# rrwick/Polypolish

Hardware: AMD Instinct MI355X
Metric: assembly Mbp polished/sec at 200x coverage; bit-identical FASTA vs reference (higher is better)
Workload: dtype u8/u32 counts + f64 depth

## Files before the change

### polypolish_amd/csrc/pp_internal.h

```cpp
#pragma once

#include <hip/hip_runtime.h>

#include <cstdarg>
#include <cstdint>
#include <cstdio>
#include <string>
#include <thread>
#include <vector>

#include "polypolish_hip.h"

#ifndef PP_MIRROR_REGISTRY_DECLARED
#define PP_MIRROR_REGISTRY_DECLARED
void pp_mirror_register_(const void *owner, const void *p, size_t bytes);
void pp_mirror_forget_(const void *owner);
bool pp_mirror_trusted_(const void *p, size_t bytes);
#endif

namespace pp {

constexpr int TILE = 2048;
constexpr int TILE_THREADS = 1024;
constexpr int COARSE_WINDOWS = 8;
// ... 122 lines not shown
    uint64_t acc_n = 0, acc_seq = 0, acc_cig = 0;
    uint64_t total_out = 0, n_multi = 0, n_keys = 0;
    uint64_t last_dev_error = ~0ull;
    std::vector<uint64_t> contig_out_off;
    std::vector<pp_contig_stats> stats;

    pp::DevBuf b_bases, b_contig_off, b_status;
    pp::DevBuf b_in[11];
    bool acc_wo = false;
    pp::DevBuf b_gstart, b_nkeep, b_aflag, b_hist, b_wincnt, b_winoff, b_entA, b_entB, b_ccnt, b_coff;
    pp::DevBuf b_code, b_winlen, b_winout, b_flag_pos, b_flag_cov, b_flag_scr, b_scratch;
    pp::DevBuf b_vote_tab;
    pp::DevBuf b_multi, b_meta, b_out, b_flag_bits, b_win_nflag, b_win_slab, b_slab_win, b_slabs, b_ents, b_keys, b_own;
    pp::DevBuf b_win_heavy, b_hslab;
    std::vector<uint64_t> wo_runs;
    pp::DevBuf b_runs, b_first, b_xcnt, b_xent, b_need_win, b_win_lo, b_win_hi;
    std::vector<uint32_t> runs_on_dev;
    size_t xcap = 0;
    bool no_direct = false;
    bool wo_untrusted = false;
    bool trust_all = false;
    bool no_wo = false;
    size_t xcap_limit = ~(size_t)0;
    uint32_t maxlen_hint = 0;
    bool last_direct = false;
    bool nothing_flagged_last = false;
    std::vector<uint32_t> emit;
    std::vector<uint32_t> run_full_of;
    uint32_t run_nc = 0;
    uint32_t last_multi = ~0u;
    uint32_t last_listed = ~0u;
// ... 73 lines not shown
```

### polypolish_amd/csrc/pp_k_direct.h

```cpp
#pragma once

#include "pp_wo_home.h"

namespace pp {

constexpr u32 NOHOME = 0xFFFFFFFFu;
__device__ __forceinline__ bool wo_bulk(bool contig_ok, u32 ref_start, u32 seq_len, u32 op0, u64 clen) {
    return contig_ok && op0 == ((seq_len << 4) | (u32)PP_OP_M) && seq_len > 0 && seq_len <= FAST_MAX_LEN && (u64)ref_start + seq_len <= clen;
}
__device__ __forceinline__ uint4 wo_item(u64 so, u32 len, u32 kc, u64 g, u32 w, u32 file_idx) {
    uint4 e;
    e.x = (u32)so;
    e.y = ((u32)(so >> 32) & 0xFFu) | (kc << 8) | (len << 24);
    e.z = (u32)(int)((long long)g - (long long)w * TILE) & 0x3FFFFFFFu;
    e.w = file_idx;
    return e;
}

constexpr u32 XLOCAL = 64, CTG_LDS = 1024;
struct CtgTab {
    const u64 *lds, *mem;
    bool in_lds;
    __device__ __forceinline__ u64 operator()(u32 i) const {
        u32 x, y;
        if (in_lds) {
            const u64 v = lds[i];
            x = (u32)v; y = (u32)(v >> 32);
            asm volatile("" : "+v"(x), "+v"(y));
        } else {
            const u64 v = mem[i];
            x = (u32)v; y = (u32)(v >> 32);
// ... 69 lines not shown
struct PrepdArgs {
    u64 n;
    const pp_wo_rec *wo;
    const u64 *cig_off;
    const u32 *n_cig, *cigar;
    const u8 *seq;
    const u64 *contig_off;
    u32 n_contigs, nwin;
    const u32 *run_end;
    u32 n_runs;
    u32 *first, *x_cnt, *x_nb;
    uint4 *xent;
    u32 xcap;
    u32 *maxlen;
    u64 *x_need;
    u64 unused_[3];
    u64 seq_bytes;
    u64 *status;
};

template <typename CTG>
__device__ __forceinline__ void general_record(const pp_wo_rec &r, const PrepdArgs &P, CTG ctg, const XSink &X) {
    u32 g_out = 0, nk_out = 0;
    u8 fl_out = 0;
    const u32 fi = r.file_idx;
    if (fi >= P.n) return;
    if (r.contig >= P.n_contigs) { report(P.status, fi, DE_BAD_CONTIG); return; }
    const u64 c_lo = ctg(r.contig), c_hi = ctg(r.contig + 1u);
    X.not_bulk(wo_home(c_lo, r.ref_start, P.nwin));
    {
        const bool multi = r.op0 == PP_WO_MULTI_RUN;
// ... 76 lines not shown
        if (lo < hi) {
            const pp_wo_rec r0 = wo[lo];
            if (r0.contig < n_contigs) wb = wo_home(P.contig_off[r0.contig], r0.ref_start, nwin);
        }
        s_wbase = wb;
    }
    XSink X{st_item, st_key, l_cnt, l_base, l_nb, &n_st, XSTAGE, 0u, P.xcap, P.x_cnt, P.x_nb, P.xent, P.x_need, status};
    X.clear();
    __syncthreads();
    PP_STAMP(0, 1);
    X.wbase = s_wbase;
    const CtgTab ctg{s_ctg, P.contig_off, ctg_lds};
    const u32 lane = threadIdx.x & 63u;
    const u32 stride = nwin + 1u;
    u32 *const first = P.first;
    auto fill = [&](bool want, u32 run, u32 from, u32 to, u32 val) {
        if (want && to - from < 4u) {
            for (u32 w = from; w <= to; w++) first[(u64)run * stride + w] = val;
            want = false;
        }
        u64 m = __ballot(want);
        while (m) {
            const int lead = __ffsll((long long)m) - 1;
            m &= m - 1;
            const u32 rr = (u32)__builtin_amdgcn_readlane((int)run, lead), ff = (u32)__builtin_amdgcn_readlane((int)from, lead),
                      tt = (u32)__builtin_amdgcn_readlane((int)to, lead), vv = (u32)__builtin_amdgcn_readlane((int)val, lead);
            for (u64 w = (u64)ff + lane; w <= tt; w += 64) first[(u64)rr * stride + w] = vv;
        }
    };
    u32 runw = 0, runw_lo = 0;
// ... 65 lines not shown
            const bool begins = valid && (starts || (hp != NOHOME && h > hp));
            const bool descent = valid && !starts && hp != NOHOME && h < hp;
            const bool ends = valid && (u32)a + 1u == run_hi;
            const bool bad = in && (file_idx >= n || k == 0 || seq_off + seq_len > (1ull << 40) || seq_off + seq_len > P.seq_bytes);
            if (__ballot(begins || descent || ends || bad)) {
                if (bad) {
                    if (file_idx >= n) report(status, a, DE_BAD_MIRROR);
                    else if (k == 0) report(status, file_idx, DE_BAD_K);
                    else if (seq_off + seq_len > (1ull << 40)) report(status, file_idx, DE_OVERFLOW);
                    else report(status, file_idx, DE_SEQ_RANGE);
                }
                if (descent) report(status, (1ull << 40) - 1ull, DE_MIRROR_ORDER);
                fill(begins, run, starts ? 0u : hp + 1u, h, (u32)a);
                fill(ends, run, h + 1u, nwin, (u32)a + 1u);
            }
            const u32 w1 = bulk ? (u32)((g + seq_len - 1u) / (u64)TILE) : 0u;
            if (bulk && w1 > h) X.emit(w1, wo_item(seq_off, seq_len, kclass_of(k), g, w1, file_idx));
            if (bulk) fast_len = max(fast_len, seq_len);
            else if (in) {
                const u32 slot = atomicAdd(&n_later, 1u);
                if (slot < LATER_MAX) { later[2u * slot] = qa[u]; later[2u * slot + 1u] = qb[u]; }
            }
            if (PP_PREPD_ROLL) ask(u, a0_next, more);
        }
        unit = unit_next;
    }
    PP_STAMP(0, 2);
    __syncthreads();
    PP_STAMP(0, 3);
    const u32 n_noted = n_later;
// ... 104 lines not shown
```

### polypolish_amd/csrc/pp_k_tile.h

```cpp
#pragma once

namespace pp {

struct TileArgs {
    const uint4 *entA;
    const u32 *win_off;
    u32 nwin;
    const u8 *seq;
    const u8 *seq4;
    const u64 *seq_off;
    const u64 *cig_off;
    const u32 *n_cig;
    const u32 *cigar;
    const u32 *kk;
    const u8 *bases;
    u64 G;
    const u64 *contig_off;
    u32 n_contigs;
    u32 min_depth;
    double fv, fi;
    u8 *code;
    u32 *win_len;
    u32 *win_coarse, *win_coarse2;
    u32 *counters;
// ... 23 lines not shown
    u64 *stamps;
#endif
    double *dbg_depth;
    u32 *dbg_counts;
    u8 *dbg_status;
    u64 *status;
    int dbg;
    const uint4 *wo;
    const u32 *first;
    u32 n_runs;
    u32 xcap;
    const u32 *x_cnt;
    const uint4 *xent;
    u32 *need_win;
    u64 *n_need;
};

struct RecMap {
    const u32 *pre;
    const u32 *first;
    u32 R;
    u32 v0, nv;
    u32 w;
    bool one_contig;
    u32 c0;
    u64 c_lo, clen;
    u32 w_in_contig;
};

struct TileShare {
    u32 b;
    u32 *any_shared;
    const u32 *kk;
    u32 *pt, *pt_over;
    const u32 *pmask;
};

__device__ __forceinline__ void share_range(u32 *cnt, u32 *ndbits, const TileShare &S, int p0, int p1, u32 kc, u32 rec) {
    if (kc == 0 || p1 <= p0) return;
    bool inexact;
    const u32 d = share_deficit(kc, S.b, S.kk, rec, &inexact);
    atomicAdd(&cnt[ROW_DEF * TILE + p0], d);
// ... 678 lines not shown
    const u32 nv_last = (u32)__builtin_amdgcn_readfirstlane((int)(nv ? nv - 1u : 0u));
    const u32 lo_w = 0u, hi_w = nv + nx;
    if (lo_w >= hi_w) return;
    auto rec_at = [&](u32 v) -> u32 {
        u32 a = M.first[0] + v;
        for (u32 r = 1; r < M.R; r++)
            if (v >= M.pre[r]) a = M.first[r] + (v - M.pre[r]);
        return a;
    };
    const uint4 *const wq = A.wo;
    auto index_of = [&](u32 u) -> u32 {
        if (REC && u < nv) return rec_at(M.v0 + r_lo + min(u, nv_last));
        const u32 x = x_lo + XS * (u - min(u, nv));
        return !REC && X.indirect ? X.indirect[x] : x;
    };
    auto words_at = [&](bool rec, u32 idx, uint4 &a, uint4 &b) {
        if (REC) {
            const uint4 *const p1 = rec ? wq + 2ull * idx : ent + idx, *const p2 = rec ? wq + 2ull * idx + 1 : ent + idx;
            a = *p1;
            b = *p2;
        } else a = ent[idx];
    };
    uint4 nxt, nxt2 = make_uint4(0, 0, 0, 0);
    {
        const u32 u = lo_w + min(lane, min(BATCH, hi_w - lo_w) - 1u);
        words_at(u < nv, index_of(u), nxt, nxt2);
    }
    for (u32 eb = lo_w; eb < hi_w; eb += BATCH) {
        const u32 nb = min(BATCH, hi_w - eb);
        uint4 my = nxt;
        bool rec_ok = true, is_rec = false;
        if (REC) {
            is_rec = eb + min(lane, nb - 1u) < nv;
            const uint4 qa = nxt, qb = nxt2;
            u64 c_lo = M.c_lo, clen = M.clen;
            bool c_ok = qa.x == M.c0;
            if (!M.one_contig) {
                const u32 cc = min(qa.x, A.n_contigs - 1u);
                c_lo = A.contig_off[cc];
                clen = A.contig_off[cc + 1] - c_lo;
                c_ok = qa.x < A.n_contigs;
            }
            rec_ok = !is_rec || wo_bulk(c_ok, qa.y, qa.w, qb.z, clen);
            const u32 kc = __ballot(is_rec && qa.z != 1u) ? kclass_of(qa.z) : 0u;
            uint4 made = wo_item((u64)qb.x | ((u64)qb.y << 32), qa.w, kc, c_lo + qa.y, M.w, qb.w);
            if (M.one_contig) made.z = (qa.y - M.w_in_contig) & 0x3FFFFFFFu;
            if (is_rec) my = made;
        }
        const bool more = eb + BATCH < hi_w;
        const u32 nxt_u = more ? eb + BATCH + min(lane, min(BATCH, hi_w - eb - BATCH) - 1u) : eb + min(lane, nb - 1u);
        const u32 nxt_idx = index_of(nxt_u);
        const bool nxt_rec = nxt_u < nv;
        auto ask_for_next = [&](u32 tie) {
            u32 idx = nxt_idx;
            asm volatile("" : "+v"(idx) : "v"(tie));
            words_at(nxt_rec, idx, nxt, nxt2);
        };
        if (!WIDE && more) ask_for_next(0u);
        const u32 my_flags = is_rec ? 0u : item_flags(my.y, my.z);
        bool my_slow = lane < nb && (my_flags & 3u) != 0;
        bool deferred = false;
        if (!REC && X.defer && __ballot(my_slow)) {
            if (my_slow) {
                const u32 slot = atomicAdd(X.defer_n, 1u);
                if (slot < X.defer_cap) {
                    X.defer[slot] = index_of(eb + lane);
                    deferred = true;
                    my_slow = false;
                }
            }
        }
// ... 113 lines not shown
    const u32 inc = wave_scan_incl(raw.len);
    const u32 total = (u32)__builtin_amdgcn_readlane((int)inc, (int)(R - 1u));
    B.pre_v = lane < R ? inc - raw.len : total;
    B.first_v = raw.f0;
    B.R = R;
    return B;
}
template <int NCH>
struct DirectBulk {
    static constexpr int GROUP_SPLIT = 5;
    BulkRuns B;
    u32 v0, nv, pm;
    const uint4 *items;
    u32 x0, nx, px;
    u32 pass;
    uint4 ea, eb;
    uint4 na, nb;
    uint4 W[NCH];
    u32 tail;
    static constexpr u32 WAVES = TILE_THREADS / 64;

    __device__ __forceinline__ u32 n_pass() const { return pm + px; }
    __device__ __forceinline__ u32 entry_of(u32 p, u32 lane) const {
        const u32 vs = v0 + 64u * p;
        const u32 v = min(vs + lane, v0 + nv - 1u);
        u32 r = 0;
        for (u32 j = 1; j < B.R; j++)
            if (vs >= (u32)__builtin_amdgcn_readlane((int)B.pre_v, (int)j)) r = j;
        u32 pr = (u32)__builtin_amdgcn_readlane((int)B.pre_v, (int)r), nx_ = (u32)__builtin_amdgcn_readlane((int)B.pre_v, (int)(r + 1u));
        u32 a = (u32)__builtin_amdgcn_readlane((int)B.first_v, (int)r) + (v - pr);
        while (__ballot(v >= nx_)) {
            r++;
            pr = nx_;
            nx_ = (u32)__builtin_amdgcn_readlane((int)B.pre_v, (int)(r + 1u));
            if (v >= pr) a = (u32)__builtin_amdgcn_readlane((int)B.first_v, (int)r) + (v - pr);
        }
        return a;
    }
    __device__ __forceinline__ void ask_sources(const TileArgs &A, u32 p, u32 lane, uint4 &qa, uint4 &qb) const {
        if (p < pm) {
            const u32 a = entry_of(p, lane);
            qa = A.wo[2ull * a];
            qb = A.wo[2ull * a + 1];
        } else {
            const u32 i = x0 + min(64u * (p - pm) + lane, nx - 1u);
            qa = items[i];
            qb = qa;
        }
    }
    __device__ __forceinline__ bool in_list(u32 p, u32 lane) const { return p < pm ? 64u * p + lane < nv : 64u * (p - pm) + lane < nx; }
    struct Lean {
        u64 so_l;
        u32 pack;
    };
    static constexpr u32 LN_REL0 = 256;
    static constexpr u32 LN_FAST = 1u << 20, LN_PLAIN = 1u << 21, LN_SHARED = 1u << 22, LN_NOTRIM = 1u << 23, LN_POINT = 1u << 24, LN_SLOW = 1u << 25;
    __device__ static __forceinline__ bool loadable(const TileArgs &A, u64 so, u32 L) {
        return L - 1u <= 32u * NCH - 1u && so + L >= 8u && so + 32u * NCH <= A.seq_bytes;
    }
    __device__ __forceinline__ Lean distill(const TileArgs &A, const RecMap &M, u32 p, const uint4 &qa, const uint4 &qb, bool listed) const {
        Lean n{0ull, 0u};
        if (p < pm) {
            const u32 ref_start = qa.y, L = qa.w;
            u32 c_lo32 = (u32)M.c_lo, clen32 = (u32)M.clen;
            bool c_ok = qa.x == M.c0;
            if (!M.one_contig) {
                const u32 cc = min(qa.x, A.n_contigs - 1u);
                const u64 lo64 = A.contig_off[cc];
                c_lo32 = (u32)lo64;
                clen32 = (u32)(A.contig_off[cc + 1] - lo64);
                c_ok = qa.x < A.n_contigs;
            }
            const u32 rel = c_lo32 + ref_start - (u32)((u64)M.w * TILE);
            const bool bulk = listed && c_ok && qb.z == ((L << 4) | (u32)PP_OP_M) && L - 1u < FAST_MAX_LEN && L <= clen32 && ref_start <= clen32 - L &&
                              rel < (u32)TILE;
            const u64 so = (u64)qb.x | ((u64)qb.y << 32);
            const bool plain = bulk && loadable(A, so, L);
            n.so_l = plain ? so : 0ull;
            n.pack = bulk ? ((rel + LN_REL0) | (L << 12) | LN_FAST | (plain ? LN_PLAIN : 0u) | (qa.z != 1u ? LN_SHARED : 0u)) : 0u;
        } else {
            const u32 ex = qa.x, ey = qa.y, ez = qa.z;
            const u32 flags = item_flags(ey, ez), L = ey >> 24;
            const bool slow = (flags & 3u) != 0, point = (flags & ENT_POINT) != 0, notrim = (flags & ENT_NOTRIM) != 0;
            const u64 so = (u64)ex | ((u64)(ey & 0xFFu) << 32);
            const int rel = item_rel(ez);
            const bool fast = listed && !slow && rel > -(int)LN_REL0 && rel < TILE;
            const bool plain = fast && !point && loadable(A, so, L) && wide4_takes(ex, ey, ez);
            n.so_l = plain ? so : 0ull;
            n.pack = listed ? (slow ? LN_SLOW : (fast ? (((u32)(rel + (int)LN_REL0)) | (L << 12) | LN_FAST | (plain ? LN_PLAIN : 0u) |
                                                         (((ey >> 8) & 0xFFu) ? LN_SHARED : 0u) | (notrim ? LN_NOTRIM : 0u) | (point ? LN_POINT : 0u))
                                                       : 0u))
                            : 0u;
        }
        return n;
    }
    __device__ __forceinline__ void begin(const TileArgs &A, const BulkRuns &runs, u32 v0_, u32 nv_, const uint4 *items_, u32 x0_, u32 nx_, u32 wave, u32 lane) {
        B = runs;
        v0 = v0_;
        nv = nv_;
        pm = (nv + 63u) >> 6;
        items = items_;
        x0 = x0_;
        nx = nx_;
        px = (nx + 63u) >> 6;
        pass = wave;
        ea = eb = make_uint4(0, 0, 0, 0);
        if (pass < n_pass()) ask_sources(A, pass, lane, ea, eb);
    }
    __device__ __forceinline__ void raw_place(const TileArgs &A, u32 p, const uint4 &qa, const uint4 &qb, u64 &so, u32 &L) const {
        if (p < pm) {
            so = (u64)qb.x | ((u64)qb.y << 32);
            L = qa.w;
        } else {
            so = (u64)qa.x | ((u64)(qa.y & 0xFFu) << 32);
            L = (qa.y & 0x00030000u) ? 0u : qa.y >> 24;
        }
    }
    __device__ __forceinline__ void stage(const TileArgs &A, u32 lane) {
        if (pass >= n_pass()) return;
        const bool more = pass + WAVES < n_pass();
        ask_sources(A, more ? pass + WAVES : pass, lane, na, nb);
        u64 so;
        u32 L;
        raw_place(A, pass, ea, eb, so, L);
        const bool ld = loadable(A, so, L);
        tail = load4_unaligned(A.seq4 + ((ld ? so + (L - 1u) : 7ull) >> 1) - 3);
        const u8 *const q = A.seq4 + ((ld ? so : 0ull) >> 1);
#pragma unroll
        for (int c = 0; c < NCH; c++) W[c] = load16_unaligned(q + 16 * c);
    }
    __device__ __forceinline__ void run(const TileArgs &A, u32 *cnt, u32 *ndbits, const TileShare &S, const u32 *asm_w, const u32 *asm4, const RecMap &M,
                                        u32 *defer, u32 *defer_n, u32 defer_cap, u32 lane) {
        const u32 np = n_pass();
        if (pass >= np) return;
        Lean cur = distill(A, M, pass, ea, eb, in_list(pass, lane));
        for (; pass < np; pass += WAVES) {
            const bool more = pass + WAVES < np;
            if (__ballot((cur.pack & (LN_SLOW | LN_POINT)) != 0 || (cur.pack & (LN_FAST | LN_PLAIN)) == LN_FAST)) {
                const int rel_r = (int)(cur.pack & 0xFFFu) - (int)LN_REL0;
                uint4 my;
                u32 src;
                if (pass < pm) {
                    src = entry_of(pass, lane);
                    const uint4 qa = A.wo[2ull * src], qb = A.wo[2ull * src + 1];
                    my = wo_item((u64)qb.x | ((u64)qb.y << 32), qa.w, kclass_of(qa.z), (u64)M.w * TILE + (u32)rel_r, M.w, qb.w);
                } else {
                    src = x0 + min(64u * (pass - pm) + lane, nx - 1u);
                    my = items[src];
                }
                if (cur.pack & LN_SLOW) {
// ... 1 lines not shown
                    if (slot < defer_cap) defer[slot] = src;
                }
                if ((cur.pack & LN_POINT) && rel_r >= 0) {
                    tile_add(cnt, (my.y >> 24) ? ROW_OTH : ROW_DEL, rel_r);
                    share_range(cnt, ndbits, S, rel_r, rel_r + 1, (my.y >> 8) & 0xFFu, my.w);
                    if ((my.y >> 24) == 2u) pt_insert(S.pt, S.pt_over, rel_r, A.seq, (u64)my.x | ((u64)(my.y & 0xFFu) << 32));
                }
                u64 rest = __ballot((cur.pack & (LN_FAST | LN_PLAIN | LN_POINT)) == LN_FAST);
                while (rest) {
                    const u32 j = (u32)__ffsll((long long)rest) - 1u;
                    rest &= rest - 1;
                    const FastItem f = fast_fetch(my, j, 64u, A.seq);
                    fast_apply(cnt, ndbits, S, asm_w, f, (u32)__builtin_amdgcn_readlane((int)my.w, (int)j), fast_load(A.seq, f, lane), lane);
                }
            }
            const Lean nxt = distill(A, M, pass + WAVES, na, nb, more && in_list(pass + WAVES, lane));
            if (pass + 2u * WAVES < np) ask_sources(A, pass + 2u * WAVES, lane, na, nb);
            const u32 tail_now = tail;
            const u8 *const q_next = A.seq4 + (nxt.so_l >> 1);
            const u8 *const t_next = A.seq4 + (((nxt.pack & LN_PLAIN) ? nxt.so_l + (((nxt.pack >> 12) & 0xFFu) - 1u) : 7ull) >> 1) - 3;

            const int rel = (int)(cur.pack & 0xFFFu) - (int)LN_REL0;
            const u32 L = (cur.pack >> 12) & 0xFFu;
            const bool plain = (cur.pack & LN_PLAIN) != 0;
            const u64 so = cur.so_l;
            const u32 adj = (u32)so & 1u;
            int nkeep = trim4(tail_now, so + (L - 1u), L);
            if (cur.pack & LN_NOTRIM) nkeep = (int)L;
            else if (plain && nkeep < 0) nkeep = trim_bytes(A.seq + so, L);
            const int lo = max(0, -rel), hi = min(nkeep, TILE - rel);
            const bool live = plain && hi > lo;
            if (live) {
// ... 221 lines not shown
        u32 inc = len;
        for (int o = 1; o < 32; o <<= 1) {
            const u32 t = (u32)__shfl_up((int)inc, o, 64);
            if ((int)r >= o) inc += t;
        }
        if (r <= R && r < 32u) s_run[r] = inc - len;
        if (r < R) s_run[32u + r] = f0;
        if (r == 63u) s_run[52] = min(A.x_cnt[w], A.xcap);
        if (r == 62u) s_run[53] = A.x_cnt[A.nwin + w];
    }
    if (tid >= 128u && tid < 128u + (u32)PMASK_WORDS) ((u32 *)s_dirty)[tid - 128u] = g_pmask_tab.v[tid - 128u];
    if (tid >= 64u && tid < 64u + PT_SLOTS * 3u) s_pt[tid - 64u] = 0;
    if (wave < 2u) {
        const u32 cw = find_contig_wave(A.contig_off, A.n_contigs, wave == 0 ? w0 : min(w0 + TILE, A.G) - 1, lane);
        if (lane == 0) { if (wave == 0) s_c0 = cw; else s_c1 = cw; }
        if (DIRECT && wave == 0 && lane == 0) {
            const u64 lo64 = A.contig_off[cw], len64 = A.contig_off[cw + 1] - lo64;
            s_run[48] = (u32)lo64; s_run[49] = (u32)(lo64 >> 32); s_run[50] = (u32)len64; s_run[51] = (u32)(len64 >> 32);
        }
    }
    if constexpr (BULK) D.stage(A, lane);
    __syncthreads();
    PP_STOP_AFTER(1)

#ifdef PP_TILE_STAMPS
    if (tid == 0) A.stamps[8ull * blockIdx.x + 6] = wall_clock64();
#endif
    u32 e0, e1, n_rec = 0, n_notbulk = 0;
    const uint4 *items;
    if (DIRECT) {
        e0 = 0;
        e1 = s_run[52];
        items = A.xent + (u64)w * A.xcap;
        n_rec = s_run[A.n_runs];
// ... 2 lines not shown
        e0 = A.win_off[w];
        e1 = A.win_off[w + 1];
        items = A.entA;
    }
    const TileShare S{win_fx_bits(e1 - e0 + n_rec - n_notbulk), &s_shared, A.kk, s_pt, &s_ptover, (const u32 *)s_dirty};
    {
        u32 i0 = e0, i1 = e1, v0 = 0, v1 = n_rec;
        if (heavy) {
            const u32 chunk = ((e1 - e0 + HEAVY_PARTS - 1u) / HEAVY_PARTS + 63u) & ~63u;
            i0 = min(e1, e0 + part * chunk);
            i1 = min(e1, i0 + chunk);
            const u32 vchunk = ((n_rec + HEAVY_PARTS - 1u) / HEAVY_PARTS + 63u) & ~63u;
            v0 = min(n_rec, part * vchunk);
            v1 = min(n_rec, v0 + vchunk);
        }
        const u32 c0 = (u32)__builtin_amdgcn_readfirstlane((int)s_c0);
        RecMap M{s_run, s_run + 32, A.n_runs, (u32)__builtin_amdgcn_readfirstlane((int)v0),
                 (u32)__builtin_amdgcn_readfirstlane((int)(v1 - v0)), w, s_c0 == s_c1, c0, 0, 0, 0};
        if (DIRECT) {
            M.c_lo = (u64)(u32)__builtin_amdgcn_readfirstlane((int)s_run[48]) | ((u64)(u32)__builtin_amdgcn_readfirstlane((int)s_run[49]) << 32);
            M.clen = (u64)(u32)__builtin_amdgcn_readfirstlane((int)s_run[50]) | ((u64)(u32)__builtin_amdgcn_readfirstlane((int)s_run[51]) << 32);
            M.w_in_contig = (u32)(w0 - M.c_lo);
        }
        constexpr u32 WAVES = TILE_THREADS / 64;
        if constexpr (BULK) {
            D.run(A, cnt, s_ndbits, S, asm_w, asm4, M, s_slow, &s_nslow, SLOW_CAP, lane);
            __syncthreads();
            const u32 n_slow = s_nslow;
            if (n_slow > SLOW_CAP) {
                const u32 n = i1 - i0;
                if (wave < n)
                    tile_items<GW, P4, false>(A, cnt, s_ndbits, S, asm_w, asm4, items, M, i0, i1,
                                              ItemList{i0 + wave, (n - wave - 1u) / WAVES + 1u, WAVES, nullptr, nullptr, nullptr, 0u, true}, wave, lane);
            } else if (wave < n_slow)
                tile_items<GW, P4, false>(A, cnt, s_ndbits, S, asm_w, asm4, items, M, i0, i1,
                                          ItemList{wave, (n_slow - wave - 1u) / WAVES + 1u, WAVES, s_slow, nullptr, nullptr, 0u, true}, wave, lane);
        } else {
            constexpr u32 IPP = (P4 && GW == 5) ? 1u : PlainCfg<GW>::IPP;
// ... 326 lines not shown
```

### polypolish_amd/csrc/pp_kernels.hip

```cpp
#include "pp_internal.h"

#include <algorithm>
#include <cstring>

#include "pp_k_common.h"
#include "pp_k_prep.h"
#include "pp_k_bucket.h"
#include "pp_k_direct.h"
#include "pp_k_tile.h"
#include "pp_k_exact.h"
#include "pp_k_emit.h"
#include "pp_k_debug.h"
#include <hip/hip_ext.h>

using namespace pp;

static bool env_is0(const char *name) { const char *v = getenv(name); return v && atoi(v) == 0; }
static bool env_on(const char *name) { const char *v = getenv(name); return v && atoi(v) != 0; }
static long env_num(const char *name, long dflt) { const char *v = getenv(name); return v ? atol(v) : dflt; }
struct Knobs {
    bool timer_record = env_on("PP_TIMER_RECORD");
    bool no_seq4 = env_is0("PP_SEQ4");
    bool no_wo = env_is0("PP_WO");
    bool no_direct = env_is0("PP_DIRECT");
// ... 548 lines not shown
    int rc;
#define ENS(buf, bytes) if ((rc = dev_ensure(ctx, ctx->buf, (size_t)(bytes)))) return rc
    ENS(b_meta, P.meta_words * 8);
    ENS(b_vote_tab, (size_t)VOTE_TAB_N * 8);
    ENS(b_win_heavy, nwin);
    ENS(b_hslab, (size_t)HEAVY_SLOTS * HEAVY_PARTS * HSLAB_WORDS * 4);
    if (!P.direct) { ENS(b_gstart, n * 4); ENS(b_nkeep, n * 4); }
    if (P.direct) {
        ENS(b_first, (uint64_t)P.n_runs * (nwin + 1) * 4);
        ENS(b_xcnt, nwin * 8);
        if (dev_ensure(ctx, ctx->b_xent, (size_t)(nwin * ctx->xcap * 16))) {
            (void)hipGetLastError();
            *no_room = true;
            return PP_OK;
        }
        ENS(b_need_win, nwin * 4); ENS(b_win_lo, nwin * 4); ENS(b_win_hi, nwin * 4);
        std::vector<uint32_t> ends(ctx->wo_runs.begin(), ctx->wo_runs.end());
        if (!(ends == ctx->runs_on_dev && ctx->b_runs.p)) {
            const void *dummy;
            ctx->runs_on_dev.clear();
            if ((rc = upload(ctx, ctx->b_runs, ends.data(), ends.size() * 4, &dummy))) return rc;
            PP_HIPCHK(ctx, hipStreamSynchronize(ctx->stream));
            ctx->runs_on_dev = ends;
        }
    }
    if (!P.direct) {
        ENS(b_hist, (uint64_t)P.NB * P.ncoarse * 4); ENS(b_wincnt, nwin * 4); ENS(b_winoff, (nwin + 1) * 4);
        ENS(b_ccnt, (uint64_t)P.ncoarse * 4); ENS(b_coff, ((uint64_t)P.ncoarse + 1) * 4);
        if (P.two_level) ENS(b_entB, ctx->cap_ent * 16);
    }
// ... 103 lines not shown
static void prep_direct(pp_ctx *ctx, const RunPlan &P, const RunDev &D) {
    const Knobs &K = knobs();
    const pp_aln_batch &B = ctx->dbatch;
    const uint64_t n = P.n;
    const u32 nwin = P.nwin;
    hipStream_t st = ctx->stream;
    const uint64_t noted_est = B.n_cig_total > n ? (B.n_cig_total - n) / 2 : 0;
    const uint64_t nbd_default = std::max<uint64_t>(std::max<uint64_t>(768, n / 8700), noted_est / 400);
    const uint32_t NBD = (uint32_t)std::max<uint64_t>(1, std::min<uint64_t>(K.prepd_blocks > 0 ? (uint64_t)K.prepd_blocks : nbd_default, (n + 2047) / 2048));
    const uint64_t chunk_d = (n + NBD - 1) / NBD;
    timer_begin(ctx, "prep");
    PrepdArgs PA{};
    PA.n = n; PA.wo = D.wo; PA.cig_off = (const u64 *)B.cig_off; PA.n_cig = B.n_cig; PA.cigar = B.cigar; PA.seq = B.seq;
    PA.contig_off = (const u64 *)ctx->b_contig_off.p; PA.n_contigs = P.nc_full; PA.nwin = nwin;
    PA.run_end = (const u32 *)ctx->b_runs.p; PA.n_runs = P.n_runs; PA.first = (u32 *)ctx->b_first.p;
    PA.x_cnt = (u32 *)ctx->b_xcnt.p; PA.x_nb = (u32 *)ctx->b_xcnt.p + nwin; PA.xent = (uint4 *)ctx->b_xent.p; PA.xcap = (u32)ctx->xcap;
    PA.maxlen = (u32 *)(D.meta + MW_MAXLEN); PA.x_need = D.meta + MW_X_NEED;
    PA.seq_bytes = B.seq_bytes;
    PA.status = D.status();
    if (K.prepd_threads == 1024) hipLaunchKernelGGL(k_prepd<1024>, dim3(NBD), dim3(1024), 0, st, (u64)chunk_d, PA);
    else hipLaunchKernelGGL(k_prepd<512>, dim3(NBD), dim3(512), 0, st, (u64)chunk_d, PA);
    timer_end(ctx);
    timer_begin(ctx, "bucket");
    hipLaunchKernelGGL(k_winplan, dim3((nwin + 255) / 256), dim3(256), 0, st, nwin, P.n_runs, (const u32 *)ctx->b_first.p,
                       (const u32 *)ctx->b_xcnt.p, (const u32 *)ctx->b_xcnt.p + nwin, (u32)ctx->xcap, P.heavy_min, D.heavy, (u8 *)ctx->b_win_heavy.p,
                       D.meta + MW_ITEMS, D.status());
    timer_end(ctx);
}

static void prep_bucketing(pp_ctx *ctx, const RunPlan &P, const RunDev &D) {
    const pp_aln_batch &B = ctx->dbatch;
// ... 87 lines not shown
    T.flag_pos = (u32 *)ctx->b_flag_pos.p; T.flag_cov = (u32 *)ctx->b_flag_cov.p;
    T.flag_bits = (u32 *)ctx->b_flag_bits.p; T.win_nflag = (u32 *)ctx->b_win_nflag.p;
    T.win_slab = (u32 *)ctx->b_win_slab.p; T.slab_win = (u32 *)ctx->b_slab_win.p; T.slabs = (u32 *)ctx->b_slabs.p; T.cap_slabs = (u32)ctx->cap_slabs;
    T.stats = (ContigStatsDev *)(D.meta + meta_stats_at(P.nc));
    T.maxlen = (const u32 *)(D.meta + MW_MAXLEN);
    T.scr_need = D.meta + MW_SCR_NEED;
    T.flag_scr = (u64 *)ctx->b_flag_scr.p;
    T.seq_bytes = B.seq_bytes;
    T.own = D.own;
    T.own_win = D.own_win;
    T.heavy = D.heavy; T.win_heavy = (u8 *)ctx->b_win_heavy.p; T.hslab = (u32 *)ctx->b_hslab.p;
    T.dbg_depth = (double *)ctx->b_dbg_depth.p; T.dbg_counts = (u32 *)ctx->b_dbg_counts.p;
    T.dbg_status = (u8 *)ctx->b_dbg_status.p; T.status = D.status();
    T.dbg = ctx->debug ? (ctx->debug_level == 3 ? 3 : (knobs().debug_replay2 ? 2 : 1)) : 0;
    T.wo = (const uint4 *)D.wo; T.first = (const u32 *)ctx->b_first.p; T.n_runs = P.n_runs; T.xcap = (u32)ctx->xcap;
    T.x_cnt = (const u32 *)ctx->b_xcnt.p; T.xent = (const uint4 *)ctx->b_xent.p; T.need_win = (u32 *)ctx->b_need_win.p; T.n_need = D.meta + MW_N_NEED;
    return T;
}

static int launch_tile(pp_ctx *ctx, const RunPlan &P, TileArgs &T) {
    hipStream_t st = ctx->stream;
    hipEvent_t ev_start = nullptr, ev_stop = nullptr;
    const bool ev_launch = timer_for_launch(ctx, "tile", &ev_start, &ev_stop);
    if (!ev_launch) timer_begin(ctx, "tile");
#ifdef PP_TILE_STAMPS
    static DevBuf b_stamps;
    const size_t stamp_bytes = (size_t)(HEAVY_BLOCKS + P.per * 8) * 64;
    if (int rc2 = dev_ensure(ctx, b_stamps, stamp_bytes)) return rc2;
    PP_HIPCHK(ctx, hipMemsetAsync(b_stamps.p, 0, stamp_bytes, st));
    T.stamps = (u64 *)b_stamps.p;
#endif
// ... 671 lines not shown

extern "C" void pp_ctx_destroy(pp_ctx *ctx) {
    if (!ctx) return;
    if (pp_ctx_wait(ctx) != PP_OK) {
        delete ctx;
        return;
    }
    pp_comm_destroy(ctx);
    (void)hipSetDevice(ctx->device);
    (void)hipStreamSynchronize(ctx->stream);
    DevBuf *all[] = {&ctx->b_comm, &ctx->b_gather, &ctx->b_bases, &ctx->b_contig_off, &ctx->b_status, &ctx->b_gstart, &ctx->b_nkeep,
                     &ctx->b_aflag, &ctx->b_hist, &ctx->b_wincnt, &ctx->b_winoff, &ctx->b_entA, &ctx->b_entB, &ctx->b_ccnt, &ctx->b_coff,
                     &ctx->b_code, &ctx->b_winlen, &ctx->b_winout, &ctx->b_flag_pos, &ctx->b_flag_cov,
                     &ctx->b_flag_scr, &ctx->b_scratch, &ctx->b_multi, &ctx->b_meta, &ctx->b_vote_tab, &ctx->b_flag_bits, &ctx->b_win_nflag, &ctx->b_win_slab, &ctx->b_slab_win, &ctx->b_slabs, &ctx->b_ents, &ctx->b_keys, &ctx->b_own,
                     &ctx->b_win_heavy, &ctx->b_hslab, &ctx->b_sub_bases,
                     &ctx->b_runs, &ctx->b_first, &ctx->b_xcnt, &ctx->b_xent, &ctx->b_need_win, &ctx->b_win_lo, &ctx->b_win_hi,
                     &ctx->b_out, &ctx->b_emit_done, &ctx->b_wincoarse, &ctx->b_dbg_depth, &ctx->b_dbg_counts, &ctx->b_dbg_status,
                     &ctx->b_dfmt_idx, &ctx->b_dfmt_rec, &ctx->b_dfmt_names, &ctx->b_dfmt_noff, &ctx->b_dfmt_emit, &ctx->b_dfmt_len,
                     &ctx->b_dfmt_bsum, &ctx->b_dfmt_boff, &ctx->b_dfmt_res, &ctx->b_dfmt_stage,
                     &ctx->f_refend[0], &ctx->f_refend[1], &ctx->f_pass[0], &ctx->f_pass[1], &ctx->f_orient, &ctx->f_poisoned,
                     &ctx->f_insert, &ctx->f_list, &ctx->f_blkcnt, &ctx->f_thr};
    for (DevBuf *b : all) dev_free(*b);
    for (auto &b : ctx->b_in) dev_free(b);
    for (auto &b : ctx->b_split) dev_free(b);
    for (auto &f : ctx->f_in) for (auto &b : f) dev_free(b);
    for (auto &b : ctx->f_rec) dev_free(b);
    timers_release(ctx);
    if (ctx->h_meta) (void)hipHostFree(ctx->h_meta);
    for (hipEvent_t e : ctx->event_pool) (void)hipEventDestroy(e);
    (void)hipStreamDestroy(ctx->stream);
    delete ctx;
// ... 46 lines not shown
```

Before: 18410.

## Precompute packed per-alignment source words in direct pass for tile kernel

The direct pass now writes a compact 8-byte source word per alignment that packs the sequence offset, window-relative position, length, and bulk/shared/far/tail flags. The tile kernel reads this word instead of two 16-byte alignment records plus contig offset lookups, which removes per-record contig bounds checks and the per-tile contig metadata in RecMap. This cuts global memory traffic and ALU work in the hot tile loop. In exchange it adds one extra buffer write per alignment in the direct pass, and shared (k!=1) records still do a gather for kclass and file index.

```diff
diff --git a/polypolish_amd/csrc/pp_internal.h b/polypolish_amd/csrc/pp_internal.h
--- a/polypolish_amd/csrc/pp_internal.h
+++ b/polypolish_amd/csrc/pp_internal.h
@@ -160,7 +160,7 @@
     pp::DevBuf b_multi, b_meta, b_out, b_flag_bits, b_win_nflag, b_win_slab, b_slab_win, b_slabs, b_ents, b_keys, b_own;
     pp::DevBuf b_win_heavy, b_hslab;
     std::vector<uint64_t> wo_runs;
-    pp::DevBuf b_runs, b_first, b_xcnt, b_xent, b_need_win, b_win_lo, b_win_hi;
+    pp::DevBuf b_runs, b_first, b_xcnt, b_xent, b_src, b_need_win, b_win_lo, b_win_hi;
     std::vector<uint32_t> runs_on_dev;
     size_t xcap = 0;
     bool no_direct = false;
diff --git a/polypolish_amd/csrc/pp_k_direct.h b/polypolish_amd/csrc/pp_k_direct.h
--- a/polypolish_amd/csrc/pp_k_direct.h
+++ b/polypolish_amd/csrc/pp_k_direct.h
@@ -15,6 +15,19 @@
     e.z = (u32)(int)((long long)g - (long long)w * TILE) & 0x3FFFFFFFu;
     e.w = file_idx;
     return e;
+}
+constexpr u32 SRC_REL_AT = 8, SRC_LEN_AT = 19, SRC_FAR_BYTES = 256;
+constexpr u32 SRC_BULK = 1u << 27;
+constexpr u32 SRC_SHARED = 1u << 28;
+constexpr u32 SRC_FAR = 1u << 29;
+constexpr u32 SRC_TAIL8 = 1u << 30;
+static_assert(TILE <= (1 << 11) && FAST_MAX_LEN < (1 << 8), "rel and the length in a source word");
+__device__ __forceinline__ uint2 wo_source(u64 so, u32 rel, u32 len, u32 k, u64 seq_bytes) {
+    uint2 s;
+    s.x = (u32)so;
+    s.y = (u32)(so >> 32) | (rel << SRC_REL_AT) | (len << SRC_LEN_AT) | SRC_BULK | (k != 1u ? SRC_SHARED : 0u) |
+          (so + SRC_FAR_BYTES <= seq_bytes ? SRC_FAR : 0u) | (so + len >= 8u ? SRC_TAIL8 : 0u);
+    return s;
 }
 
 constexpr u32 XLOCAL = 64, CTG_LDS = 1024;
@@ -114,7 +127,8 @@
     u32 xcap;
     u32 *maxlen;
     u64 *x_need;
-    u64 unused_[3];
+    uint2 *src;
+    u64 unused_[2];
     u64 seq_bytes;
     u64 *status;
 };
@@ -221,6 +235,7 @@
     const u32 lane = threadIdx.x & 63u;
     const u32 stride = nwin + 1u;
     u32 *const first = P.first;
+    uint2 *const src = P.src;
     auto fill = [&](bool want, u32 run, u32 from, u32 to, u32 val) {
         if (want && to - from < 4u) {
             for (u32 w = from; w <= to; w++) first[(u64)run * stride + w] = val;
@@ -316,6 +331,7 @@
                 fill(begins, run, starts ? 0u : hp + 1u, h, (u32)a);
                 fill(ends, run, h + 1u, nwin, (u32)a + 1u);
             }
+            if (in) src[a] = bulk && !bad ? wo_source(seq_off, (u32)g - h * (u32)TILE, seq_len, k, P.seq_bytes) : make_uint2(0u, 0u);
             const u32 w1 = bulk ? (u32)((g + seq_len - 1u) / (u64)TILE) : 0u;
             if (bulk && w1 > h) X.emit(w1, wo_item(seq_off, seq_len, kclass_of(k), g, w1, file_idx));
             if (bulk) fast_len = max(fast_len, seq_len);
diff --git a/polypolish_amd/csrc/pp_k_tile.h b/polypolish_amd/csrc/pp_k_tile.h
--- a/polypolish_amd/csrc/pp_k_tile.h
+++ b/polypolish_amd/csrc/pp_k_tile.h
@@ -61,6 +61,7 @@
     const uint4 *xent;
     u32 *need_win;
     u64 *n_need;
+    const uint2 *src;
 };
 
 struct RecMap {
@@ -69,10 +70,6 @@
     u32 R;
     u32 v0, nv;
     u32 w;
-    bool one_contig;
-    u32 c0;
-    u64 c_lo, clen;
-    u32 w_in_contig;
 };
 
 struct TileShare {
@@ -781,17 +778,17 @@
         const u32 x = x_lo + XS * (u - min(u, nv));
         return !REC && X.indirect ? X.indirect[x] : x;
     };
-    auto words_at = [&](bool rec, u32 idx, uint4 &a, uint4 &b) {
+    auto words_at = [&](bool rec, u32 idx, uint4 &a) {
         if (REC) {
-            const uint4 *const p1 = rec ? wq + 2ull * idx : ent + idx, *const p2 = rec ? wq + 2ull * idx + 1 : ent + idx;
-            a = *p1;
-            b = *p2;
+            const uint2 *const p1 = rec ? A.src + idx : (const uint2 *)(ent + idx), *const p2 = rec ? p1 : p1 + 1;
+            const uint2 lo = *p1, hi = *p2;
+            a = make_uint4(lo.x, lo.y, hi.x, hi.y);
         } else a = ent[idx];
     };
-    uint4 nxt, nxt2 = make_uint4(0, 0, 0, 0);
+    uint4 nxt;
     {
         const u32 u = lo_w + min(lane, min(BATCH, hi_w - lo_w) - 1u);
-        words_at(u < nv, index_of(u), nxt, nxt2);
+        words_at(u < nv, index_of(u), nxt);
     }
     for (u32 eb = lo_w; eb < hi_w; eb += BATCH) {
         const u32 nb = min(BATCH, hi_w - eb);
@@ -799,19 +796,17 @@
         bool rec_ok = true, is_rec = false;
         if (REC) {
             is_rec = eb + min(lane, nb - 1u) < nv;
-            const uint4 qa = nxt, qb = nxt2;
-            u64 c_lo = M.c_lo, clen = M.clen;
-            bool c_ok = qa.x == M.c0;
-            if (!M.one_contig) {
-                const u32 cc = min(qa.x, A.n_contigs - 1u);
-                c_lo = A.contig_off[cc];
-                clen = A.contig_off[cc + 1] - c_lo;
-                c_ok = qa.x < A.n_contigs;
-            }
-            rec_ok = !is_rec || wo_bulk(c_ok, qa.y, qa.w, qb.z, clen);
-            const u32 kc = __ballot(is_rec && qa.z != 1u) ? kclass_of(qa.z) : 0u;
-            uint4 made = wo_item((u64)qb.x | ((u64)qb.y << 32), qa.w, kc, c_lo + qa.y, M.w, qb.w);
-            if (M.one_contig) made.z = (qa.y - M.w_in_contig) & 0x3FFFFFFFu;
+            const u32 sy = nxt.y;
+            rec_ok = !is_rec || (sy & SRC_BULK) != 0;
+            u32 kc = 0, fi = 0;
+            if (__ballot(is_rec && (sy & SRC_SHARED) != 0)) {
+                if (is_rec && (sy & SRC_SHARED) != 0) {
+                    const u32 idx = index_of(eb + min(lane, nb - 1u));
+                    kc = kclass_of(wq[2ull * idx].z);
+                    fi = wq[2ull * idx + 1].w;
+                }
+            }
+            const uint4 made = make_uint4(nxt.x, (sy & 0xFFu) | (kc << 8) | (((sy >> SRC_LEN_AT) & 0xFFu) << 24), (sy >> SRC_REL_AT) & (u32)(TILE - 1), fi);
             if (is_rec) my = made;
         }
         const bool more = eb + BATCH < hi_w;
@@ -821,7 +816,7 @@
         auto ask_for_next = [&](u32 tie) {
             u32 idx = nxt_idx;
             asm volatile("" : "+v"(idx) : "v"(tie));
-            words_at(nxt_rec, idx, nxt, nxt2);
+            words_at(nxt_rec, idx, nxt);
         };
         if (!WIDE && more) ask_for_next(0u);
         const u32 my_flags = is_rec ? 0u : item_flags(my.y, my.z);
@@ -965,8 +960,8 @@
     const uint4 *items;
     u32 x0, nx, px;
     u32 pass;
-    uint4 ea, eb;
-    uint4 na, nb;
+    uint4 ea;
+    uint4 na;
     uint4 W[NCH];
     u32 tail;
     static constexpr u32 WAVES = TILE_THREADS / 64;
@@ -988,17 +983,18 @@
         }
         return a;
     }
-    __device__ __forceinline__ void ask_sources(const TileArgs &A, u32 p, u32 lane, uint4 &qa, uint4 &qb) const {
+    __device__ __forceinline__ void ask_sources(const TileArgs &A, u32 p, u32 lane, uint4 &q) const {
         if (p < pm) {
-            const u32 a = entry_of(p, lane);
-            qa = A.wo[2ull * a];
-            qb = A.wo[2ull * a + 1];
+            const uint2 s = A.src[entry_of(p, lane)];
+            q = make_uint4(s.x, s.y, 0u, 0u);
         } else {
             const u32 i = x0 + min(64u * (p - pm) + lane, nx - 1u);
-            qa = items[i];
-            qb = qa;
-        }
-    }
+            q = items[i];
+        }
+    }
+    __device__ static __forceinline__ u64 src_so(const uint4 &q) { return (u64)q.x | ((u64)(q.y & 0xFFu) << 32); }
+    __device__ static __forceinline__ u32 src_len(const uint4 &q) { return (q.y >> SRC_LEN_AT) & 0xFFu; }
+    __device__ static __forceinline__ u32 src_rel(const uint4 &q) { return (q.y >> SRC_REL_AT) & (u32)(TILE - 1); }
     __device__ __forceinline__ bool in_list(u32 p, u32 lane) const { return p < pm ? 64u * p + lane < nv : 64u * (p - pm) + lane < nx; }
     struct Lean {
         u64 so_l;
@@ -1009,26 +1005,17 @@
     __device__ static __forceinline__ bool loadable(const TileArgs &A, u64 so, u32 L) {
         return L - 1u <= 32u * NCH - 1u && so + L >= 8u && so + 32u * NCH <= A.seq_bytes;
     }
-    __device__ __forceinline__ Lean distill(const TileArgs &A, const RecMap &M, u32 p, const uint4 &qa, const uint4 &qb, bool listed) const {
+    static_assert(32u * NCH <= SRC_FAR_BYTES, "SRC_FAR covers the instance's chunk loads");
+    __device__ static __forceinline__ bool src_loadable(const TileArgs &A, const uint4 &q) {
+        return src_len(q) - 1u <= 32u * NCH - 1u && (q.y & SRC_TAIL8) != 0 && ((q.y & SRC_FAR) != 0 || src_so(q) + 32u * NCH <= A.seq_bytes);
+    }
+    __device__ __forceinline__ Lean distill(const TileArgs &A, u32 p, const uint4 &qa, bool listed) const {
         Lean n{0ull, 0u};
         if (p < pm) {
-            const u32 ref_start = qa.y, L = qa.w;
-            u32 c_lo32 = (u32)M.c_lo, clen32 = (u32)M.clen;
-            bool c_ok = qa.x == M.c0;
-            if (!M.one_contig) {
-                const u32 cc = min(qa.x, A.n_contigs - 1u);
-                const u64 lo64 = A.contig_off[cc];
-                c_lo32 = (u32)lo64;
-                clen32 = (u32)(A.contig_off[cc + 1] - lo64);
-                c_ok = qa.x < A.n_contigs;
-            }
-            const u32 rel = c_lo32 + ref_start - (u32)((u64)M.w * TILE);
-            const bool bulk = listed && c_ok && qb.z == ((L << 4) | (u32)PP_OP_M) && L - 1u < FAST_MAX_LEN && L <= clen32 && ref_start <= clen32 - L &&
-                              rel < (u32)TILE;
-            const u64 so = (u64)qb.x | ((u64)qb.y << 32);
-            const bool plain = bulk && loadable(A, so, L);
-            n.so_l = plain ? so : 0ull;
-            n.pack = bulk ? ((rel + LN_REL0) | (L << 12) | LN_FAST | (plain ? LN_PLAIN : 0u) | (qa.z != 1u ? LN_SHARED : 0u)) : 0u;
+            const bool bulk = listed && (qa.y & SRC_BULK) != 0;
+            const bool plain = bulk && src_loadable(A, qa);
+            n.so_l = plain ? src_so(qa) : 0ull;
+            n.pack = bulk ? ((src_rel(qa) + LN_REL0) | (src_len(qa) << 12) | LN_FAST | (plain ? LN_PLAIN : 0u) | ((qa.y & SRC_SHARED) ? LN_SHARED : 0u)) : 0u;
         } else {
             const u32 ex = qa.x, ey = qa.y, ez = qa.z;
             const u32 flags = item_flags(ey, ez), L = ey >> 24;
@@ -1055,26 +1042,26 @@
         nx = nx_;
         px = (nx + 63u) >> 6;
         pass = wave;
-        ea = eb = make_uint4(0, 0, 0, 0);
-        if (pass < n_pass()) ask_sources(A, pass, lane, ea, eb);
-    }
-    __device__ __forceinline__ void raw_place(const TileArgs &A, u32 p, const uint4 &qa, const uint4 &qb, u64 &so, u32 &L) const {
+        ea = make_uint4(0, 0, 0, 0);
+        if (pass < n_pass()) ask_sources(A, pass, lane, ea);
+    }
+    __device__ __forceinline__ bool raw_place(const TileArgs &A, u32 p, const uint4 &qa, u64 &so, u32 &L) const {
         if (p < pm) {
-            so = (u64)qb.x | ((u64)qb.y << 32);
-            L = qa.w;
-        } else {
-            so = (u64)qa.x | ((u64)(qa.y & 0xFFu) << 32);
-            L = (qa.y & 0x00030000u) ? 0u : qa.y >> 24;
-        }
+            so = src_so(qa);
+            L = src_len(qa);
+            return src_loadable(A, qa);
+        }
+        so = (u64)qa.x | ((u64)(qa.y & 0xFFu) << 32);
+        L = (qa.y & 0x00030000u) ? 0u : qa.y >> 24;
+        return loadable(A, so, L);
     }
     __device__ __forceinline__ void stage(const TileArgs &A, u32 lane) {
         if (pass >= n_pass()) return;
         const bool more = pass + WAVES < n_pass();
-        ask_sources(A, more ? pass + WAVES : pass, lane, na, nb);
+        ask_sources(A, more ? pass + WAVES : pass, lane, na);
         u64 so;
         u32 L;
-        raw_place(A, pass, ea, eb, so, L);
-        const bool ld = loadable(A, so, L);
+        const bool ld = raw_place(A, pass, ea, so, L);
         tail = load4_unaligned(A.seq4 + ((ld ? so + (L - 1u) : 7ull) >> 1) - 3);
         const u8 *const q = A.seq4 + ((ld ? so : 0ull) >> 1);
 #pragma unroll
@@ -1084,7 +1071,7 @@
                                         u32 *defer, u32 *defer_n, u32 defer_cap, u32 lane) {
         const u32 np = n_pass();
         if (pass >= np) return;
-        Lean cur = distill(A, M, pass, ea, eb, in_list(pass, lane));
+        Lean cur = distill(A, pass, ea, in_list(pass, lane));
         for (; pass < np; pass += WAVES) {
             const bool more = pass + WAVES < np;
             if (__ballot((cur.pack & (LN_SLOW | LN_POINT)) != 0 || (cur.pack & (LN_FAST | LN_PLAIN)) == LN_FAST)) {
@@ -1116,8 +1103,8 @@
                     fast_apply(cnt, ndbits, S, asm_w, f, (u32)__builtin_amdgcn_readlane((int)my.w, (int)j), fast_load(A.seq, f, lane), lane);
                 }
             }
-            const Lean nxt = distill(A, M, pass + WAVES, na, nb, more && in_list(pass + WAVES, lane));
-            if (pass + 2u * WAVES < np) ask_sources(A, pass + 2u * WAVES, lane, na, nb);
+            const Lean nxt = distill(A, pass + WAVES, na, more && in_list(pass + WAVES, lane));
+            if (pass + 2u * WAVES < np) ask_sources(A, pass + 2u * WAVES, lane, na);
             const u32 tail_now = tail;
             const u8 *const q_next = A.seq4 + (nxt.so_l >> 1);
             const u8 *const t_next = A.seq4 + (((nxt.pack & LN_PLAIN) ? nxt.so_l + (((nxt.pack >> 12) & 0xFFu) - 1u) : 7ull) >> 1) - 3;
@@ -1369,10 +1356,6 @@
     if (wave < 2u) {
         const u32 cw = find_contig_wave(A.contig_off, A.n_contigs, wave == 0 ? w0 : min(w0 + TILE, A.G) - 1, lane);
         if (lane == 0) { if (wave == 0) s_c0 = cw; else s_c1 = cw; }
-        if (DIRECT && wave == 0 && lane == 0) {
-            const u64 lo64 = A.contig_off[cw], len64 = A.contig_off[cw + 1] - lo64;
-            s_run[48] = (u32)lo64; s_run[49] = (u32)(lo64 >> 32); s_run[50] = (u32)len64; s_run[51] = (u32)(len64 >> 32);
-        }
     }
     if constexpr (BULK) D.stage(A, lane);
     __syncthreads();
@@ -1405,14 +1388,8 @@
             v0 = min(n_rec, part * vchunk);
             v1 = min(n_rec, v0 + vchunk);
         }
-        const u32 c0 = (u32)__builtin_amdgcn_readfirstlane((int)s_c0);
-        RecMap M{s_run, s_run + 32, A.n_runs, (u32)__builtin_amdgcn_readfirstlane((int)v0),
-                 (u32)__builtin_amdgcn_readfirstlane((int)(v1 - v0)), w, s_c0 == s_c1, c0, 0, 0, 0};
-        if (DIRECT) {
-            M.c_lo = (u64)(u32)__builtin_amdgcn_readfirstlane((int)s_run[48]) | ((u64)(u32)__builtin_amdgcn_readfirstlane((int)s_run[49]) << 32);
-            M.clen = (u64)(u32)__builtin_amdgcn_readfirstlane((int)s_run[50]) | ((u64)(u32)__builtin_amdgcn_readfirstlane((int)s_run[51]) << 32);
-            M.w_in_contig = (u32)(w0 - M.c_lo);
-        }
+        const RecMap M{s_run, s_run + 32, A.n_runs, (u32)__builtin_amdgcn_readfirstlane((int)v0),
+                       (u32)__builtin_amdgcn_readfirstlane((int)(v1 - v0)), w};
         constexpr u32 WAVES = TILE_THREADS / 64;
         if constexpr (BULK) {
             D.run(A, cnt, s_ndbits, S, asm_w, asm4, M, s_slow, &s_nslow, SLOW_CAP, lane);
diff --git a/polypolish_amd/csrc/pp_kernels.hip b/polypolish_amd/csrc/pp_kernels.hip
--- a/polypolish_amd/csrc/pp_kernels.hip
+++ b/polypolish_amd/csrc/pp_kernels.hip
@@ -586,6 +586,7 @@
             *no_room = true;
             return PP_OK;
         }
+        ENS(b_src, n * 8);
         ENS(b_need_win, nwin * 4); ENS(b_win_lo, nwin * 4); ENS(b_win_hi, nwin * 4);
         std::vector<uint32_t> ends(ctx->wo_runs.begin(), ctx->wo_runs.end());
         if (!(ends == ctx->runs_on_dev && ctx->b_runs.p)) {
@@ -719,7 +720,7 @@
     PA.n = n; PA.wo = D.wo; PA.cig_off = (const u64 *)B.cig_off; PA.n_cig = B.n_cig; PA.cigar = B.cigar; PA.seq = B.seq;
     PA.contig_off = (const u64 *)ctx->b_contig_off.p; PA.n_contigs = P.nc_full; PA.nwin = nwin;
     PA.run_end = (const u32 *)ctx->b_runs.p; PA.n_runs = P.n_runs; PA.first = (u32 *)ctx->b_first.p;
-    PA.x_cnt = (u32 *)ctx->b_xcnt.p; PA.x_nb = (u32 *)ctx->b_xcnt.p + nwin; PA.xent = (uint4 *)ctx->b_xent.p; PA.xcap = (u32)ctx->xcap;
+    PA.x_cnt = (u32 *)ctx->b_xcnt.p; PA.x_nb = (u32 *)ctx->b_xcnt.p + nwin; PA.xent = (uint4 *)ctx->b_xent.p; PA.xcap = (u32)ctx->xcap; PA.src = (uint2 *)ctx->b_src.p;
     PA.maxlen = (u32 *)(D.meta + MW_MAXLEN); PA.x_need = D.meta + MW_X_NEED;
     PA.seq_bytes = B.seq_bytes;
     PA.status = D.status();
@@ -837,7 +838,7 @@
     T.dbg_status = (u8 *)ctx->b_dbg_status.p; T.status = D.status();
     T.dbg = ctx->debug ? (ctx->debug_level == 3 ? 3 : (knobs().debug_replay2 ? 2 : 1)) : 0;
     T.wo = (const uint4 *)D.wo; T.first = (const u32 *)ctx->b_first.p; T.n_runs = P.n_runs; T.xcap = (u32)ctx->xcap;
-    T.x_cnt = (const u32 *)ctx->b_xcnt.p; T.xent = (const uint4 *)ctx->b_xent.p; T.need_win = (u32 *)ctx->b_need_win.p; T.n_need = D.meta + MW_N_NEED;
+    T.x_cnt = (const u32 *)ctx->b_xcnt.p; T.xent = (const uint4 *)ctx->b_xent.p; T.src = (const uint2 *)ctx->b_src.p; T.need_win = (u32 *)ctx->b_need_win.p; T.n_need = D.meta + MW_N_NEED;
     return T;
 }
 
@@ -1539,7 +1540,7 @@
                      &ctx->b_code, &ctx->b_winlen, &ctx->b_winout, &ctx->b_flag_pos, &ctx->b_flag_cov,
                      &ctx->b_flag_scr, &ctx->b_scratch, &ctx->b_multi, &ctx->b_meta, &ctx->b_vote_tab, &ctx->b_flag_bits, &ctx->b_win_nflag, &ctx->b_win_slab, &ctx->b_slab_win, &ctx->b_slabs, &ctx->b_ents, &ctx->b_keys, &ctx->b_own,
                      &ctx->b_win_heavy, &ctx->b_hslab, &ctx->b_sub_bases,
-                     &ctx->b_runs, &ctx->b_first, &ctx->b_xcnt, &ctx->b_xent, &ctx->b_need_win, &ctx->b_win_lo, &ctx->b_win_hi,
+                     &ctx->b_runs, &ctx->b_first, &ctx->b_xcnt, &ctx->b_xent, &ctx->b_src, &ctx->b_need_win, &ctx->b_win_lo, &ctx->b_win_hi,
                      &ctx->b_out, &ctx->b_emit_done, &ctx->b_wincoarse, &ctx->b_dbg_depth, &ctx->b_dbg_counts, &ctx->b_dbg_status,
                      &ctx->b_dfmt_idx, &ctx->b_dfmt_rec, &ctx->b_dfmt_names, &ctx->b_dfmt_noff, &ctx->b_dfmt_emit, &ctx->b_dfmt_len,
                      &ctx->b_dfmt_bsum, &ctx->b_dfmt_boff, &ctx->b_dfmt_res, &ctx->b_dfmt_stage,
```

Result: faster. 18790 (median of 6 runs) (+2.0%).
